# mrlooi/PoseCNN

Hardware: AMD Instinct MI355X
Metric: frames/sec 640x480x21-class Hough-vote+RoI+ADD-loss, 1/2/4/8 MI355X (higher is better)
Workload: dtype f32 (FC GEMMs: exact 3-way split-bf16 x6 MFMA, products within 2^-24, fp32 accumulate: fp32-faithful)

## Files before the change

include/posecnn_hip.h:

```cpp
#ifndef POSECNN_HIP_H
#define POSECNN_HIP_H

#include <stddef.h>
#include <stdint.h>

#ifdef __cplusplus
extern "C" {
#endif

#define PCNN_OK 0
#define PCNN_EINVAL 1
#define PCNN_EHIP 2
#define PCNN_ECAPACITY 3

#define PCNN_MAX_ROI 128

int pcnn_abi_version(void);
const char* pcnn_strerror(int code);

int pcnn_set_completion_event(void* event);
int pcnn_completion_event_pending(void);

size_t pcnn_hough_voting_workspace_size(int B, int H, int W, int C, int skip_pixels, float vote_thr);

// ... 36 lines not shown
                           float scale_b, int B, int C, const float* rois, int R_cap, int roi_stride,
                           int batch_base, const int32_t* num_rois_dev, int pooled_h, int pooled_w, float* top_sum,
                           int32_t* argmax_a, int32_t* argmax_b, void* stream);

int pcnn_roi_pool_fwd_pair_px(const float* data_a, int Ha, int Wa, float scale_a, const float* data_b, int Hb,
                              int Wb, float scale_b, int B, int C, const float* rois, int R_cap, int roi_stride,
                              int batch_base, const int32_t* num_rois_dev, int pooled_h, int pooled_w,
                              float* top_sum, uint16_t* argmax_a, uint16_t* argmax_b, void* stream);

size_t pcnn_roi_pool_bwd_workspace_size(int B, int R_cap);

int pcnn_roi_pool_bwd_form(int B, int H, int W, int C, int layout, int pool_channel, int pooled_h, int pooled_w,
                           int R_cap, int px);

int pcnn_roi_pool_bwd(const float* top_diff, const int32_t* argmax, int B, int H, int W, int C, int layout,
                      const float* rois, int R_cap, int roi_stride, int batch_base, const int32_t* num_rois_dev,
                      float spatial_scale, int pooled_h, int pooled_w, int pool_channel, float* bottom_diff,
                      void* workspace, size_t workspace_bytes, void* stream);

int pcnn_roi_pool_bwd_px(const float* top_diff, const uint16_t* argmax_px, int B, int H, int W, int C,
                         const float* rois, int R_cap, int roi_stride, int batch_base, const int32_t* num_rois_dev,
                         float spatial_scale, int pooled_h, int pooled_w, float* bottom_diff, void* workspace,
                         size_t workspace_bytes, void* stream);

size_t pcnn_add_loss_workspace_size(int R_cap, int C, int P);
size_t pcnn_add_loss_stats_offset(int R_cap, int C, int P);

int pcnn_add_loss_fwd(const float* pred, const float* target, const float* weight, const float* points,
                      const float* symmetry, int R_cap, const int32_t* num_rois_dev, int C, int P, float margin,
                      int loss_norm_rows, const int32_t* loss_norm_rows_dev, float* loss, float* bottom_diff,
                      void* workspace, size_t workspace_bytes, void* stream);

int pcnn_add_loss_prep(const float* weight, const float* symmetry, int R_cap, const int32_t* num_rois_dev, int C,
                       int P, void* workspace, size_t workspace_bytes, void* stream);
int pcnn_add_loss_fwd_prepared(const float* pred, const float* target, const float* weight, const float* points,
                               const float* symmetry, int R_cap, const int32_t* num_rois_dev, int C, int P,
                               float margin, int loss_norm_rows, const int32_t* loss_norm_rows_dev, float* loss,
                               float* bottom_diff, void* workspace, size_t workspace_bytes, void* stream);

int pcnn_add_loss_fwd_head_bwd(const float* pred, const float* target, const float* weight, const float* points,
                               const float* symmetry, int R_cap, const int32_t* num_rois_dev, int C, int P,
                               float margin, int loss_norm_rows, const int32_t* loss_norm_rows_dev,
                               float* bottom_diff, void* workspace, size_t workspace_bytes, const float* tanh_out,
                               const float* d_pred_scale, float* d_y8, void* stream);
int pcnn_add_loss_total(int R_cap, const int32_t* num_rois_dev, int C, int P, const void* workspace,
                        size_t workspace_bytes, float* loss, void* stream);
// ... 197 lines not shown
```

posecnn_amd/_lib.py:

```python
import ctypes
import os
import threading

import torch

_HERE = os.path.dirname(os.path.abspath(__file__))
LIB_PATH = os.environ.get("POSECNN_HIP_LIB") or os.path.join(_HERE, "libposecnn_hip.so")

_lib = None
_lock = threading.Lock()

c_int = ctypes.c_int
c_float = ctypes.c_float
c_size_t = ctypes.c_size_t
c_void_p = ctypes.c_void_p

_SIGS = {
    "pcnn_abi_version": (c_int, []),
    "pcnn_strerror": (ctypes.c_char_p, [c_int]),
    "pcnn_set_completion_event": (c_int, [c_void_p]),
    "pcnn_completion_event_pending": (c_int, []),
    "pcnn_hough_voting_workspace_size": (c_size_t, [c_int, c_int, c_int, c_int, c_int, c_float]),
    "pcnn_hough_voting": (c_int, [c_void_p, c_void_p, c_void_p, c_void_p, c_int, c_void_p, c_int, c_int, c_int,
                                  c_int, c_int, c_int, c_int, c_int, c_float, c_int, c_float, c_float, c_int,
# ... 5 lines not shown
                                       c_int, c_void_p, c_void_p, c_size_t, c_void_p]),
    "pcnn_hough_voting_compact": (c_int, [c_void_p, c_void_p, c_void_p, c_void_p, c_int, c_void_p, c_int, c_int,
                                          c_int, c_int, c_int, c_int, c_int, c_int, c_float, c_int, c_float, c_float,
                                          c_int, c_void_p, c_void_p, c_void_p, c_void_p, c_void_p, c_void_p, c_int,
                                          c_void_p, c_void_p, c_size_t, c_void_p]),
    "pcnn_hough_voting_grad": (c_int, [c_void_p, c_void_p, c_int, c_int, c_int, c_int, c_void_p]),
    "pcnn_hough_voting_diag": (c_int, [c_void_p, c_int, c_int, c_int, c_int, c_int, c_float, c_void_p, c_void_p]),
    "pcnn_roi_pool_fwd": (c_int, [c_void_p, c_int, c_int, c_int, c_int, c_int, c_void_p, c_int, c_int, c_int,
                                  c_void_p, c_float, c_int, c_int, c_int, c_void_p, c_void_p, c_void_p]),
    "pcnn_roi_pool_fwd_accumulate": (c_int, [c_void_p, c_int, c_int, c_int, c_int, c_int, c_void_p, c_int, c_int,
                                             c_int, c_void_p, c_float, c_int, c_int, c_int, c_void_p, c_void_p, c_void_p]),
    "pcnn_roi_pool_fwd_pair": (c_int, [c_void_p, c_int, c_int, c_float, c_void_p, c_int, c_int, c_float, c_int, c_int,
                                       c_void_p, c_int, c_int, c_int, c_void_p, c_int, c_int, c_void_p, c_void_p,
                                       c_void_p, c_void_p]),
    "pcnn_roi_pool_fwd_pair_px": (c_int, [c_void_p, c_int, c_int, c_float, c_void_p, c_int, c_int, c_float, c_int,
                                          c_int, c_void_p, c_int, c_int, c_int, c_void_p, c_int, c_int, c_void_p,
                                          c_void_p, c_void_p, c_void_p]),
    "pcnn_roi_pool_bwd_workspace_size": (c_size_t, [c_int, c_int]),
    "pcnn_roi_pool_bwd_form": (c_int, [c_int, c_int, c_int, c_int, c_int, c_int, c_int, c_int, c_int, c_int]),
    "pcnn_roi_pool_bwd_px": (c_int, [c_void_p, c_void_p, c_int, c_int, c_int, c_int, c_void_p, c_int, c_int, c_int,
                                     c_void_p, c_float, c_int, c_int, c_void_p, c_void_p, c_size_t, c_void_p]),
    "pcnn_roi_pool_bwd": (c_int, [c_void_p, c_void_p, c_int, c_int, c_int, c_int, c_int, c_void_p, c_int, c_int,
                                  c_int, c_void_p, c_float, c_int, c_int, c_int, c_void_p, c_void_p, c_size_t, c_void_p]),
    "pcnn_add_loss_workspace_size": (c_size_t, [c_int, c_int, c_int]),
    "pcnn_add_loss_stats_offset": (c_size_t, [c_int, c_int, c_int]),
    "pcnn_add_loss_fwd": (c_int, [c_void_p, c_void_p, c_void_p, c_void_p, c_void_p, c_int, c_void_p, c_int, c_int,
                                  c_float, c_int, c_void_p, c_void_p, c_void_p, c_void_p, c_size_t, c_void_p]),
    "pcnn_add_loss_fwd_prepared": (c_int, [c_void_p, c_void_p, c_void_p, c_void_p, c_void_p, c_int, c_void_p, c_int, c_int,
                                  c_float, c_int, c_void_p, c_void_p, c_void_p, c_void_p, c_size_t, c_void_p]),
    "pcnn_add_loss_prep": (c_int, [c_void_p, c_void_p, c_int, c_void_p, c_int, c_int, c_void_p, c_size_t, c_void_p]),
    "pcnn_add_loss_fwd_head_bwd": (c_int, [c_void_p, c_void_p, c_void_p, c_void_p, c_void_p, c_int, c_void_p, c_int,
                                           c_int, c_float, c_int, c_void_p, c_void_p, c_void_p, c_size_t, c_void_p,
                                           c_void_p, c_void_p, c_void_p]),
    "pcnn_add_loss_total": (c_int, [c_int, c_void_p, c_int, c_int, c_void_p, c_size_t, c_void_p, c_void_p]),
    "pcnn_add_loss_bwd": (c_int, [c_void_p, c_void_p, c_int, c_void_p, c_int, c_void_p, c_void_p]),
    "pcnn_div_rn_check": (c_int, [c_void_p, c_float, c_int, c_int, c_void_p, c_void_p]),
    "pcnn_backproject_fwd": (c_int, [c_void_p, c_void_p, c_void_p, c_void_p, c_int, c_void_p, c_int, c_int, c_int,
                                     c_int, c_int, c_int, c_int, c_float, c_void_p, c_void_p, c_void_p, c_void_p]),
    "pcnn_backproject_bwd": (c_int, [c_void_p, c_void_p, c_void_p, c_int, c_int, c_int, c_int, c_int, c_int,
                                     c_void_p, c_void_p]),
    "pcnn_gemm_workspace_size": (c_size_t, [c_int, c_int, c_int, c_int, c_int]),
    "pcnn_gemm": (c_int, [c_int, c_int, c_int, c_void_p, c_void_p, c_int, c_int, c_void_p, c_int, c_int, c_void_p,
                          c_int, c_void_p, c_int, c_void_p, c_int, c_void_p, c_void_p, c_int, c_void_p, c_size_t,
                          c_void_p]),
    "pcnn_gemm_drop": (c_int, [c_int, c_int, c_int, c_void_p, c_void_p, c_int, c_int, c_void_p, c_int, c_int,
                               c_void_p, c_int, c_void_p, c_int, c_void_p, c_int, c_void_p, c_int, c_float, c_void_p,
# ... 186 lines not shown
```

posecnn_amd/csrc/roi_plan.h:

```cpp
#pragma once

namespace pcnn_roi {

#ifndef PCNN_RBW_NARROW
#define PCNN_RBW_NARROW 8192
#endif
#ifndef PCNN_RBW_TH
#define PCNN_RBW_TH 2
#endif
static_assert(PCNN_RBW_TH == 1 || PCNN_RBW_TH == 2, "the entry-list forms are 1x4 and 2x4");

constexpr int kBWaves = 1;
constexpr int kBChunk = 128 * kBWaves;
constexpr int kBTileW = 4;
constexpr int kBGroup = 16;
constexpr int kBBins = 49;
constexpr int kBCap = kBGroup * kBBins;

enum BwdForm { kBwdRejected = -1, kBwdGeneric = 0, kBwdEnt1x4 = 1, kBwdEnt2x4 = 2 };

struct BwdPlan {
  int form;
  int tbh;
};
// ... 5 lines not shown
inline int bwd_tile_h(int B, int H, int W, int C) {
  const long nchunk = ((long)C + kBChunk - 1) / kBChunk;
  const long wg24 = (long)B * (((long)H + 1) / 2) * (((long)W + 3) / 4) * nchunk;
  return wg24 < PCNN_RBW_NARROW ? 1 : PCNN_RBW_TH;
}

inline BwdPlan bwd_plan(int B, int H, int W, int C, int layout, int pool_channel, int pooled_h, int pooled_w,
                        int R_cap, int px) {
  BwdPlan p = {kBwdRejected, 0};
  if (B <= 0 || H <= 0 || W <= 0 || C <= 0 || pooled_h <= 0 || pooled_w <= 0 || R_cap < 0 ||
      (layout != 0 && layout != 1) || !map_below(H, W, C, 1l << 31))
    return p;
  const int tbh = bwd_tile_h(B, H, W, C);
  const long bins = (long)pooled_h * pooled_w;
  const bool ent = layout == 0 && !pool_channel && C % 2 == 0 && (long)pooled_h * tbh <= 32 &&
                   (long)pooled_w * kBTileW <= 32 && kBGroup * bins <= kBCap && map_below(H, W, C, 1l << 30) &&
                   R_cap <= ((1l << 29) - 1) / (bins * C);
  if (px && !(ent && (long)H * W < 0xFFFF)) return p;
  p.form = !ent ? kBwdGeneric : tbh == 1 ? kBwdEnt1x4 : kBwdEnt2x4;
  p.tbh = ent ? tbh : 0;
  return p;
}

}
```

posecnn_amd/csrc/roi_pooling.hip:

```cpp
#include "pcnn_common.h"
#include "roi_plan.h"
#include <math.h>
#include <cfloat>

namespace {


struct RoiGeo {
  int b, cls, sw, sh, ew, eh;
  float bin_h, bin_w;
};

__device__ __forceinline__ RoiGeo roi_geo(const float* __restrict__ rois, int r, int stride, int batch_base,
                                          float scale, int PH, int PW) {
  const float* o = rois + (size_t)r * stride;
  RoiGeo g;
  g.b = (int)o[0] - batch_base;
  const int c0 = stride == 5 ? 1 : 2;
  g.cls = stride == 5 ? 0 : (int)o[1];
  g.sw = (int)roundf(o[c0 + 0] * scale);
  g.sh = (int)roundf(o[c0 + 1] * scale);
  g.ew = (int)roundf(o[c0 + 2] * scale);
  g.eh = (int)roundf(o[c0 + 3] * scale);
  const int roi_w = max(g.ew - g.sw + 1, 1);
// ... 365 lines not shown
        }
      };
      if (total > 0) {
        int2 myA, myB, avA[kBBatch], avB[kBBatch];
        float2 dvA[kBBatch], dvB[kBBatch];
        fetch(0, myA, avA, dvA);
        for (int e0 = 0; e0 < total; e0 += 2 * kBBatch) {
          if (e0 + kBBatch < total) fetch(e0 + kBBatch, myB, avB, dvB);
          accumulate(e0, myA, avA, dvA);
          if (e0 + 2 * kBBatch < total) fetch(e0 + 2 * kBBatch, myA, avA, dvA);
          if (e0 + kBBatch < total) accumulate(e0 + kBBatch, myB, avB, dvB);
        }
      }
      __syncthreads();
    }
  }
  if (cok) {
#pragma unroll
    for (int i = 0; i < kBTH; i++)
#pragma unroll
      for (int j = 0; j < kBTW; j++)
        if (i < th && j < tw) *(float2*)(bottom + (((size_t)b * H + h0 + i) * W + w0 + j) * C + c) = acc[i * kBTW + j];
  }
}

__global__ void k_roi_bwd_generic(const float* __restrict__ top_diff, const int32_t* __restrict__ argmax, int B,
                                  int H, int W, int C, int layout, const int32_t* __restrict__ geo, int PH, int PW,
                                  int pool_channel, const int32_t* __restrict__ lo, const int32_t* __restrict__ hi,
                                  float* __restrict__ bottom) {
  const long npix = (long)B * H * W;
  const int Co = pool_channel ? 1 : C;
  for (long pi = (long)blockIdx.x * blockDim.x + threadIdx.x; pi < npix; pi += (long)gridDim.x * blockDim.x) {
    const int w = (int)(pi % W), h = (int)((pi / W) % H), b = (int)(pi / ((long)W * H));
    const int r0 = lo[b], r1 = hi[b];
    for (int r = r0; r <= r1; r++) {
      const int32_t* gg = geo + (size_t)r * 8;
      RoiGeo g;
      g.b = gg[0]; g.cls = gg[1]; g.sw = gg[2]; g.sh = gg[3]; g.ew = gg[4]; g.eh = gg[5];
      g.bin_h = __int_as_float(gg[6]);
      g.bin_w = __int_as_float(gg[7]);
      if (g.b != b) continue;
      if (!(w >= g.sw && w <= g.ew && h >= g.sh && h <= g.eh)) continue;
      int phs, phe, pws, pwe;
      bins_of_pixel(g, h, w, PH, PW, phs, phe, pws, pwe);
      const int cb = pool_channel ? g.cls : 0, ce = pool_channel ? g.cls + 1 : C;
      if (cb < 0 || ce > C) continue;
// ... 162 lines not shown
    const int blocks = (int)((npix + 255) / 256 < 8192 ? (npix + 255) / 256 : 8192);
    hipLaunchKernelGGL(k_roi_bwd_generic, dim3(blocks), dim3(256), 0, st, top_diff, (const int32_t*)argmax, B, H, W,
                       C, layout, geo, pooled_h, pooled_w, pool_channel, lo, hi, bottom_diff);
  }
  PCNN_CHECK_LAUNCH();
  return PCNN_OK;
}

extern "C" int pcnn_roi_pool_bwd(const float* top_diff, const int32_t* argmax, int B, int H, int W, int C, int layout,
                                 const float* rois, int R_cap, int roi_stride, int batch_base,
                                 const int32_t* num_rois_dev, float spatial_scale, int pooled_h, int pooled_w,
                                 int pool_channel, float* bottom_diff, void* workspace, size_t workspace_bytes, void* stream) {
  return roi_pool_bwd(top_diff, argmax, false, B, H, W, C, layout, rois, R_cap, roi_stride, batch_base, num_rois_dev,
                      spatial_scale, pooled_h, pooled_w, pool_channel, bottom_diff, workspace, workspace_bytes, stream);
}

extern "C" int pcnn_roi_pool_bwd_px(const float* top_diff, const uint16_t* argmax_px, int B, int H, int W, int C,
                                    const float* rois, int R_cap, int roi_stride, int batch_base,
                                    const int32_t* num_rois_dev, float spatial_scale, int pooled_h, int pooled_w,
                                    float* bottom_diff, void* workspace, size_t workspace_bytes, void* stream) {
  return roi_pool_bwd(top_diff, argmax_px, true, B, H, W, C, 0, rois, R_cap, roi_stride, batch_base, num_rois_dev,
                      spatial_scale, pooled_h, pooled_w, 0, bottom_diff, workspace, workspace_bytes, stream);
}
```

posecnn_amd/pipeline.py:

```python
import contextlib

import torch

from . import _lib
from . import pose_head as ph
from .hough_voting_gpu_layer import hough_voting_gpu_op as hv
from .roi_pooling_layer import roi_pooling_op as rp
from .average_distance_loss import average_distance_loss_op as adl
from .exchange import GradShard, RoiExchange

CAP = hv.CAPACITY
_nullctx = contextlib.nullcontext


class PoseStep:
    def __init__(self, B, H, W, num_classes, device, conv4_hw=None, conv5_hw=None, channels=512, units=4096,
                 is_train=1, skip_pixels=10, vote_threshold=-1.0, vote_percentage=0.02, margin=0.01,
                 global_batch=None, batch_base=0, weights=None, dist=None, backward=True, precision=2,
                 overlap_weight_grads=True, pixel_argmax=True, keep_prob=None, drop_seed=0x5EED, side_prep=True,
                 drop_in_reduce=True, pipeline=False, prefetch_at="loss", fuse_loss_tail=True,
                 defer_side_join=False, signal_forks=True, pool_at_tail=False, fuse_fc8=True):
        self.B, self.H, self.W, self.C = B, H, W, num_classes
        self.dev = device
        self.is_train, self.skip, self.vthr, self.vper, self.margin = is_train, skip_pixels, vote_threshold, \
            vote_percentage, margin
        self.global_batch = global_batch or B
        self.batch_base = batch_base
        self.dist = dist
        self.backward = backward
        self.prec = precision
        self.h4, self.w4 = conv4_hw or (H // 8, W // 8)
        self.h5, self.w5 = conv5_hw or (H // 16, W // 16)
        self.Ch = channels
        D = 4 * num_classes
        self.D = D
        self.fuse_fc8 = bool(fuse_fc8) and dist is None and ph.fc8_fused_ok(units, D, precision) and D % 4 == 0
        self.weights = weights or ph.PoseHeadWeights(num_classes, device, in_dim=49 * channels, units=units)
        f32 = dict(dtype=torch.float32, device=device)
        i32 = dict(dtype=torch.int32, device=device)
        K6 = 49 * channels
        px = pixel_argmax and max(self.h4 * self.w4, self.h5 * self.w5) < 0xFFFF
        adt = dict(dtype=torch.int16 if px else torch.int32, device=device)

        def minibatch_set():
            return dict(hough=dict(box=torch.zeros((CAP, 7), **f32), pose=torch.zeros((CAP, 7), **f32),
                                   target=torch.zeros((CAP, D), **f32), weight=torch.zeros((CAP, D), **f32),
                                   domain=torch.zeros((CAP,), **i32), num_rois=torch.zeros((2,), **i32)),
                        pool=torch.zeros((CAP, 7, 7, channels), **f32),
                        arg5=torch.zeros((CAP, 7, 7, channels), **adt),
                        arg4=torch.zeros((CAP, 7, 7, channels), **adt),
                        add_ws=None, prepped=False)
        self.fuse_loss_tail = fuse_loss_tail
        self.pipeline = bool(pipeline)
        self._sets = [minibatch_set() for _ in range(2 if self.pipeline else 1)]
        self._cur = 0
        self._primed = None
        self.prefetch_at = prefetch_at
        if prefetch_at not in ("loss", "bwd", "start", "fwd", "tail"):
            raise ValueError("prefetch_at must be 'start', 'fwd', 'loss', 'bwd' or 'tail'")
        self._fork_ev = torch.cuda.Event() if self.pipeline else None
        self._fork_recorded = False
        self.pre_stream = torch.cuda.Stream(device=device) if self.pipeline else None
        self._next = None
        self.y6 = torch.zeros((CAP, units), **f32)
        self.y7 = torch.zeros((CAP, units), **f32)
        self.y8 = torch.zeros((CAP, D), **f32)
        self.t8 = torch.zeros((CAP, D), **f32)
        self.pred = torch.zeros((CAP, D), **f32)
        self.loss = torch.zeros((1,), **f32)
        self.diff = torch.zeros((CAP, D), **f32)
        self.one = torch.ones((1,), **f32)
        self.dy8 = torch.zeros((CAP, D), **f32)
        self.dy7 = torch.zeros((CAP, units), **f32)
        self.dy6 = torch.zeros((CAP, units), **f32)
        self.dx = torch.zeros((CAP, K6), **f32)
        self.gshard = None
        if dist is not None:
            per_max = 9 if is_train else 1
            slot = max(1, min(CAP, B * (hv.MAX_ROI // self.global_batch) * per_max))
            self.gshard = GradShard(dist, slot, [("w6", (K6, units)), ("w7", (units, units)), ("w8", (units, D))],
                                    device)
        self.grads = self.weights.grads_like()
        if self.gshard is not None:
            for k in ("w6", "w7", "w8"):
                self.grads[k] = self.grads[k][self.gshard.rows(k)].contiguous()
        self.keep = float(keep_prob if keep_prob is not None else (0.5 if is_train else 1.0))
# ... 105 lines not shown
        s = self._cur if s is None else s
        st = self._sets[s]
        if st["add_ws"] is None:
            st["add_ws"] = torch.empty(adl.workspace_bytes(CAP, self.C, points.shape[1]), dtype=torch.uint8,
                                       device=self.dev)
        h = st["hough"]
        side = None
        if stream is None:
            side = self.side_stream if self.timer is None and self.side_prep else None
            if side is not None:
                side.wait_stream(torch.cuda.current_stream())
        with torch.cuda.stream(stream or side or torch.cuda.current_stream()):
            adl.average_distance_loss_prep(h["weight"], symmetry, points.shape[1], st["add_ws"],
                                           num_rois=h["num_rois"][1:2])
        st["prepped"] = "side" if side is not None else "stream"

    def pool_fwd(self, conv4, conv5, s=None):
        s = self._cur if s is None else s
        st = self._sets[s]
        with self._t("roi_pool_fwd"):
            rp.roi_pool_pair(conv5, 1.0 / 16.0, conv4, 1.0 / 8.0, st["hough"]["box"], 7, 7,
                             num_rois=st["hough"]["num_rois"][1:2], out=(st["pool"], st["arg5"], st["arg4"]),
                             batch_base=self.batch_base)
        st["pooled"] = True

    def _front(self, inputs, s, stream=None):
        ctx = torch.cuda.stream(stream) if stream is not None else _nullctx()
        with ctx:
            self.vote(inputs["label"], inputs["vertex"], inputs["extents"], inputs["meta"], inputs["gt"], s=s)
            if stream is not None:
                self.add_prep(inputs["points"], inputs["symmetry"], s=s, stream=stream)
                if self.pool_at_tail and stream is self.pre_stream:
                    self._pool_pending = (inputs, s)
                else:
                    self.pool_fwd(inputs["conv4"], inputs["conv5"], s=s)

    def _issue_pending_pool(self):
        if self._pool_pending is None:
            return
        inputs, s = self._pool_pending
        self._pool_pending = None
        with torch.cuda.stream(self.pre_stream):
            self.pool_fwd(inputs["conv4"], inputs["conv5"], s=s)

    def _prefetch(self):
        if self._next is None:
# ... 185 lines not shown
        self._head_bwd_done = False
        if self.prefetch_at == "bwd":
            self._prefetch()
        with self._t("gemm_fc8_fc7_dw_bias"):
            weight_grads("w8", self.y7, self.dy8, CAP, w.units, self.D, fork=not fused_fork)
        dk = dict(keep_prob=self.keep) if self.keep < 1.0 else {}
        ev = self._arm_fork("fc8_dx") if side is not None else None
        with self._t("gemm_fc8_fc7_dx"):
            if self.fuse_fc8:
                self._timed_gemm("fc8_dx", lambda: ph.fc8_dx(self.dy8, w.w8, self.dy7, mask=self.y7, M_dev=nr,
                                                             precision=self.prec, **dk))
            else:
                self._g("fc8_dx", self.dy8, w.w8, self.dy7, b_trans=1, mask=self.y7, M_dev=nr, **dk)
        ev = self._fork_taken(ev)
        with self._t("gemm_fc8_fc7_dw_bias"):
            weight_grads("w7", self.y6, self.dy7, CAP, w.units, w.units, fork_ev=ev)
        defer = self.defer_side_join and side is not None
        self._side_wait("_side_done_ev")
        self._side_pending = False
        if defer:
            self._mid_covers_pre = (self._primed is not None and self._pool_pending is None and
                                    not torch.cuda.is_current_stream_capturing())
            if self._mid_covers_pre:
                side.wait_stream(self.pre_stream)
            if self._bump_drop_step and self._mid_covers_pre:
                with torch.cuda.stream(side):
                    self.drop_step.add_(1)
                self._bump_drop_step = False
            self._side_mid_ev.record(side)
        ev = self._arm_fork("fc7_dx") if side is not None else None
        with self._t("gemm_fc8_fc7_dx"):
            self._g("fc7_dx", self.dy7, w.w7, self.dy6, b_trans=1, mask=self.y6, M_dev=nr, **dk)
        ev = self._fork_taken(ev)
        with self._t("gemm_fc6_dw"):
            weight_grads("w6", x, self.dy6, CAP, K6, w.units, fork_ev=ev)
        with self._t("gemm_fc6_dx"):
            self._g("fc6_dx", self.dy6, w.w6, self.dx, b_trans=1, M_dev=nr)
        if self.prefetch_at == "tail":
            self._prefetch()
        self._issue_pending_pool()
        dxp = self.dx.view(CAP, 7, 7, self.Ch)
        with self._t("roi_pool_bwd"):
            rp.roi_pool_grad(conv5, h["box"], self.arg5, dxp, 7, 7, 1.0 / 16.0, 0, num_rois=nr, out=self.dconv5,
                             batch_base=self.batch_base)
            rp.roi_pool_grad(conv4, h["box"], self.arg4, dxp, 7, 7, 1.0 / 8.0, 0, num_rois=nr, out=self.dconv4,
                             batch_base=self.batch_base)
        if self._bump_drop_step:
            self.drop_step.add_(1)
            self._bump_drop_step = False
        if defer:
            self._side_done_ev.record(side)
            self._side_pending = True
        elif side is not None:
            main.wait_stream(side)

    def _g(self, name, A, B, C, **kw):
        self._timed_gemm(name, lambda: ph.gemm(A, B, C, precision=self.prec, **kw))
        return C

    def _timed_gemm(self, name, launch):
        if self.gemm_timer is None:
            return launch()
        e0, e1 = torch.cuda.Event(enable_timing=True), torch.cuda.Event(enable_timing=True)
        e0.record()
        out = launch()
        e1.record()
        self.gemm_timer.setdefault(name, []).append((e0, e1))
        return out

# ... 56 lines not shown
```

posecnn_amd/roi_pooling_layer/roi_pooling_op.py:

```python
import torch

from .. import _lib


def roi_pool(bottom_data, bottom_rois, pooled_height, pooled_width, spatial_scale, pool_channel=0, name=None,
             num_rois=None, layout=0, out=None, accumulate=False, batch_base=0):
    _lib.require_gpu(bottom_data, bottom_rois)
    if bottom_data.dim() != 4:
        raise ValueError("data must be 4-dimensional")
    if bottom_rois.dim() != 2:
        raise ValueError("rois must be 2-dimensional")
    data = bottom_data.contiguous().float()
    rois = bottom_rois.contiguous().float()
    if layout == 0:
        B, H, W, C = data.shape
    else:
        B, C, H, W = data.shape
    R, stride = rois.shape
    Co = 1 if pool_channel else C
    shape = (R, pooled_height, pooled_width, Co) if layout == 0 else (R, Co, pooled_height, pooled_width)
    if out is None:
        if accumulate:
            raise ValueError("accumulate=True needs out=(top, argmax)")
        top = torch.empty(shape, dtype=torch.float32, device=data.device)
# ... 53 lines not shown
    R, stride = rois.shape
    lib = _lib.load()
    ws = _lib.workspace(lib.pcnn_roi_pool_bwd_workspace_size(B, R), bottom_data.device, "roi_bwd")
    dd = out if out is not None else torch.empty(bottom_data.shape, dtype=torch.float32, device=bottom_data.device)
    px = argmax.dtype == torch.int16
    if R == 0:
        rois = argmax = grad = ws
    if px:
        if layout != 0 or pool_channel:
            raise ValueError("a pixel-index argmax needs NHWC data and pool_channel 0")
        rc = lib.pcnn_roi_pool_bwd_px(_lib.ptr(grad.contiguous()), _lib.ptr(argmax.contiguous()), B, H, W, C,
                                      _lib.ptr(rois), R, stride, int(batch_base), _lib.ptr(num_rois),
                                      float(spatial_scale), int(pooled_height), int(pooled_width), _lib.ptr(dd),
                                      _lib.ptr(ws), ws.numel(), _lib.stream_ptr())
    else:
        rc = lib.pcnn_roi_pool_bwd(_lib.ptr(grad.contiguous()), _lib.ptr(argmax.contiguous()), B, H, W, C, layout,
                                   _lib.ptr(rois), R, stride, int(batch_base), _lib.ptr(num_rois),
                                   float(spatial_scale), int(pooled_height), int(pooled_width), int(pool_channel),
                                   _lib.ptr(dd), _lib.ptr(ws), ws.numel(), _lib.stream_ptr())
    _lib.check(rc, "roi_pool_grad")
    return dd


class RoiPoolFunction(torch.autograd.Function):

    @staticmethod
    def forward(ctx, data, rois, pooled_height, pooled_width, spatial_scale, pool_channel=0, layout=0):
        top, arg = roi_pool(data, rois, pooled_height, pooled_width, spatial_scale, pool_channel, layout=layout)
        ctx.save_for_backward(data, rois, arg)
        ctx.params = (pooled_height, pooled_width, spatial_scale, pool_channel, layout)
        return top, arg

    @staticmethod
    def backward(ctx, grad, _garg):
        data, rois, arg = ctx.saved_tensors
        ph, pw, sc, pc, layout = ctx.params
        return roi_pool_grad(data, rois, arg, grad, ph, pw, sc, pc, layout=layout), None, None, None, None, None, None
```

Baseline: 4604.

## Precompute RoI-pool backward tile plan on prefetch stream and fuse conv4/conv5 backward

Adds a plan step that builds per-tile lists of intersecting RoIs with bin row and column bitmasks, using a count pass, a prefix scan and a fill pass. The step is issued after forward RoI pooling, on the prefetch stream when pipelining is on. The backward pass then walks only the precomputed records, skipping the per-tile RoI geometry scan, and runs conv4 and conv5 in a single paired launch with double-buffered loads. The cost is extra plan buffers, three small extra kernels per step and event synchronisation between streams; if the plan cannot be hidden on the side stream, it adds work to the step.

```diff
diff --git a/include/posecnn_hip.h b/include/posecnn_hip.h
--- a/include/posecnn_hip.h
+++ b/include/posecnn_hip.h
@@ -82,6 +82,20 @@
                          const float* rois, int R_cap, int roi_stride, int batch_base, const int32_t* num_rois_dev,
                          float spatial_scale, int pooled_h, int pooled_w, float* bottom_diff, void* workspace,
                          size_t workspace_bytes, void* stream);
+
+size_t pcnn_roi_pool_bwd_plan_bytes(int B, int H, int W, int C, int pooled_h, int pooled_w, int R_cap);
+int pcnn_roi_pool_bwd_plan(int B, int H, int W, int C, const float* rois, int R_cap, int roi_stride, int batch_base,
+                           const int32_t* num_rois_dev, float spatial_scale, int pooled_h, int pooled_w, void* plan,
+                           size_t plan_bytes, void* stream);
+
+int pcnn_roi_pool_bwd_planned(const float* top_diff, const void* argmax, int px, int B, int H, int W, int C,
+                              int R_cap, int pooled_h, int pooled_w, const void* plan, size_t plan_bytes,
+                              float* bottom_diff, void* stream);
+
+int pcnn_roi_pool_bwd_planned_pair(const float* top_diff, int px, int B, int C, int R_cap, int pooled_h, int pooled_w,
+                                   const void* argmax_a, int Ha, int Wa, const void* plan_a, size_t plan_a_bytes,
+                                   float* bottom_a, const void* argmax_b, int Hb, int Wb, const void* plan_b,
+                                   size_t plan_b_bytes, float* bottom_b, void* stream);
 
 size_t pcnn_add_loss_workspace_size(int R_cap, int C, int P);
 size_t pcnn_add_loss_stats_offset(int R_cap, int C, int P);
diff --git a/posecnn_amd/_lib.py b/posecnn_amd/_lib.py
--- a/posecnn_amd/_lib.py
+++ b/posecnn_amd/_lib.py
@@ -51,6 +51,14 @@
                                      c_void_p, c_float, c_int, c_int, c_void_p, c_void_p, c_size_t, c_void_p]),
     "pcnn_roi_pool_bwd": (c_int, [c_void_p, c_void_p, c_int, c_int, c_int, c_int, c_int, c_void_p, c_int, c_int,
                                   c_int, c_void_p, c_float, c_int, c_int, c_int, c_void_p, c_void_p, c_size_t, c_void_p]),
+    "pcnn_roi_pool_bwd_plan_bytes": (c_size_t, [c_int, c_int, c_int, c_int, c_int, c_int, c_int]),
+    "pcnn_roi_pool_bwd_plan": (c_int, [c_int, c_int, c_int, c_int, c_void_p, c_int, c_int, c_int, c_void_p, c_float,
+                                       c_int, c_int, c_void_p, c_size_t, c_void_p]),
+    "pcnn_roi_pool_bwd_planned": (c_int, [c_void_p, c_void_p, c_int, c_int, c_int, c_int, c_int, c_int, c_int, c_int,
+                                          c_void_p, c_size_t, c_void_p, c_void_p]),
+    "pcnn_roi_pool_bwd_planned_pair": (c_int, [c_void_p, c_int, c_int, c_int, c_int, c_int, c_int,
+                                               c_void_p, c_int, c_int, c_void_p, c_size_t, c_void_p,
+                                               c_void_p, c_int, c_int, c_void_p, c_size_t, c_void_p, c_void_p]),
     "pcnn_add_loss_workspace_size": (c_size_t, [c_int, c_int, c_int]),
     "pcnn_add_loss_stats_offset": (c_size_t, [c_int, c_int, c_int]),
     "pcnn_add_loss_fwd": (c_int, [c_void_p, c_void_p, c_void_p, c_void_p, c_void_p, c_int, c_void_p, c_int, c_int,
diff --git a/posecnn_amd/csrc/roi_plan.h b/posecnn_amd/csrc/roi_plan.h
--- a/posecnn_amd/csrc/roi_plan.h
+++ b/posecnn_amd/csrc/roi_plan.h
@@ -1,4 +1,7 @@
 #pragma once
+#include <math.h>
+#include <stddef.h>
+#include <stdint.h>
 
 namespace pcnn_roi {
 
@@ -51,4 +54,78 @@
   return p;
 }
 
+
+#if defined(__HIP__) || defined(__HIPCC__)
+#define PCNN_ROI_HD __host__ __device__
+#else
+#define PCNN_ROI_HD
+#endif
+
+PCNN_ROI_HD inline bool tile_hit(int sw, int sh, int ew, int eh, float bin_h, float bin_w, int h0, int w0, int th,
+                                 int tw, int tbh, int PH, int PW, uint32_t& rbits, uint32_t& cbits) {
+  rbits = 0;
+  cbits = 0;
+  if (!(sh <= h0 + th - 1 && eh >= h0 && sw <= w0 + tw - 1 && ew >= w0)) return false;
+  for (int i = 0; i < th; i++) {
+    const int h = h0 + i;
+    if (h < sh || h > eh) continue;
+    int s0 = (int)floorf((float)(h - sh) / bin_h), e0 = (int)ceilf((float)(h - sh + 1) / bin_h);
+    s0 = s0 < 0 ? 0 : (s0 > PH ? PH : s0);
+    e0 = e0 < 0 ? 0 : (e0 > PH ? PH : e0);
+    for (int ph = s0; ph < e0; ph++) rbits |= 1u << (ph * tbh + i);
+  }
+  for (int j = 0; j < tw; j++) {
+    const int w = w0 + j;
+    if (w < sw || w > ew) continue;
+    int s0 = (int)floorf((float)(w - sw) / bin_w), e0 = (int)ceilf((float)(w - sw + 1) / bin_w);
+    s0 = s0 < 0 ? 0 : (s0 > PW ? PW : s0);
+    e0 = e0 < 0 ? 0 : (e0 > PW ? PW : e0);
+    for (int pw = s0; pw < e0; pw++) cbits |= 1u << (pw * kBTileW + j);
+  }
+  return rbits != 0 && cbits != 0;
 }
+
+constexpr int kPlanRowBits = 20;
+PCNN_ROI_HD inline uint64_t plan_pack(uint32_t r, uint32_t rbits, uint32_t cbits, int rb, int cb) {
+  return (uint64_t)cbits | ((uint64_t)rbits << cb) | ((uint64_t)r << (cb + rb));
+}
+PCNN_ROI_HD inline void plan_unpack(uint64_t rec, int rb, int cb, uint32_t& r, uint32_t& rbits, uint32_t& cbits) {
+  cbits = (uint32_t)(rec & ((1ull << cb) - 1));
+  rbits = (uint32_t)((rec >> cb) & ((1ull << rb) - 1));
+  r = (uint32_t)(rec >> (cb + rb));
+}
+
+constexpr int kPlanMagic = 0x524f4950;
+constexpr int kPlanHdr = 8;
+
+struct PlanLayout {
+  int ok, tbh;
+  long tpi, tiles, cap;
+  size_t hdr, lo, hi, geo, off, rec, bytes;
+};
+
+inline size_t plan_align(size_t x) { return (x + 255) / 256 * 256; }
+
+inline PlanLayout plan_layout(int B, int H, int W, int C, int pooled_h, int pooled_w, int R_cap) {
+  PlanLayout L = {};
+  const BwdPlan p = bwd_plan(B, H, W, C, 0, 0, pooled_h, pooled_w, R_cap, 0);
+  if (p.form != kBwdEnt1x4 && p.form != kBwdEnt2x4) return L;
+  if (R_cap >= (1 << kPlanRowBits) || pooled_h * p.tbh + pooled_w * kBTileW + kPlanRowBits > 64) return L;
+  L.tbh = p.tbh;
+  L.tpi = (((long)H + p.tbh - 1) / p.tbh) * (((long)W + kBTileW - 1) / kBTileW);
+  L.tiles = (long)B * L.tpi;
+  L.cap = (long)R_cap * L.tpi;
+  if (L.cap >= (1l << 31) || L.tiles >= (1l << 31) - 1) return L;
+  size_t o = 0;
+  L.hdr = o; o = plan_align(o + kPlanHdr * 4);
+  L.lo = o;  o = plan_align(o + (size_t)B * 4);
+  L.hi = o;  o = plan_align(o + (size_t)B * 4);
+  L.geo = o; o = plan_align(o + (size_t)(R_cap > 0 ? R_cap : 1) * 32);
+  L.off = o; o = plan_align(o + (size_t)(L.tiles + 1) * 4);
+  L.rec = o; o = plan_align(o + (size_t)(L.cap > 0 ? L.cap : 1) * 8);
+  L.bytes = o;
+  L.ok = 1;
+  return L;
+}
+
+}
diff --git a/posecnn_amd/csrc/roi_pooling.hip b/posecnn_amd/csrc/roi_pooling.hip
--- a/posecnn_amd/csrc/roi_pooling.hip
+++ b/posecnn_amd/csrc/roi_pooling.hip
@@ -411,6 +411,232 @@
       for (int j = 0; j < kBTW; j++)
         if (i < th && j < tw) *(float2*)(bottom + (((size_t)b * H + h0 + i) * W + w0 + j) * C + c) = acc[i * kBTW + j];
   }
+}
+
+
+template <bool FILL>
+__global__ void __launch_bounds__(256) k_roi_plan_tiles(const int32_t* __restrict__ geo,
+                                                         const int32_t* __restrict__ lo,
+                                                         const int32_t* __restrict__ hi, int H, int W, int tbh,
+                                                         int PH, int PW, int tpi, int tiles,
+                                                         int32_t* __restrict__ off, uint64_t* __restrict__ recs) {
+  const int tile = (int)blockIdx.x * 4 + (int)(threadIdx.x >> 6);
+  if (tile >= tiles) return;
+  const int lane = pcnn::lane_id();
+  const int tiles_w = (W + pcnn_roi::kBTileW - 1) / pcnn_roi::kBTileW;
+  const int b = tile / tpi, t = tile % tpi;
+  const int h0 = (t / tiles_w) * tbh, w0 = (t % tiles_w) * pcnn_roi::kBTileW;
+  const int th = min(tbh, H - h0), tw = min(pcnn_roi::kBTileW, W - w0);
+  const int r0 = lo[b], r1 = hi[b];
+  const int base = FILL ? off[tile] : 0;
+  int n = 0;
+  for (int rb = r0; rb <= r1; rb += 64) {
+    const int r = rb + lane;
+    uint32_t rbits = 0, cbits = 0;
+    bool hit = false;
+    if (r <= r1) {
+      const int32_t* gg = geo + (size_t)r * 8;
+      if (gg[0] == b)
+        hit = pcnn_roi::tile_hit(gg[2], gg[3], gg[4], gg[5], __int_as_float(gg[6]), __int_as_float(gg[7]), h0, w0, th,
+                                 tw, tbh, PH, PW, rbits, cbits);
+    }
+    const uint64_t hits = __ballot(hit);
+    if (FILL && hit)
+      recs[(size_t)base + n + __popcll(hits & pcnn::lanemask_lt())] =
+          pcnn_roi::plan_pack((uint32_t)r, rbits, cbits, PH * tbh, PW * pcnn_roi::kBTileW);
+    n += __popcll(hits);
+  }
+  if (!FILL && lane == 0) off[tile] = n;
+}
+
+__global__ void __launch_bounds__(1024) k_roi_plan_scan(int32_t* __restrict__ off, int tiles, int32_t* __restrict__ hdr,
+                                                         int B, int H, int W, int tbh, int PH, int PW, int R_cap) {
+  __shared__ int wsum[16];
+  const int lane = pcnn::lane_id(), wave = threadIdx.x >> 6;
+  int carry = 0;
+  for (int t0 = 0; t0 < tiles; t0 += 1024) {
+    const int i = t0 + (int)threadIdx.x;
+    const int v = i < tiles ? off[i] : 0;
+    int s = v;
+#pragma unroll
+    for (int d = 1; d < 64; d <<= 1) {
+      const int u = __shfl_up(s, d, 64);
+      if (lane >= d) s += u;
+    }
+    if (lane == 63) wsum[wave] = s;
+    __syncthreads();
+    int before = 0, total = 0;
+#pragma unroll
+    for (int k = 0; k < 16; k++) {
+      const int ws = wsum[k];
+      before += k < wave ? ws : 0;
+      total += ws;
+    }
+    if (i < tiles) off[i] = carry + before + s - v;
+    carry += total;
+    __syncthreads();
+  }
+  if (threadIdx.x == 0) {
+    off[tiles] = carry;
+    hdr[0] = pcnn_roi::kPlanMagic; hdr[1] = B; hdr[2] = H; hdr[3] = W;
+    hdr[4] = tbh; hdr[5] = PH; hdr[6] = PW; hdr[7] = R_cap;
+  }
+}
+
+struct PlanMap {
+  const void* argmax;
+  const int32_t* hdr;
+  const int32_t* off;
+  const uint64_t* recs;
+  float* bottom;
+  int H, W;
+  int items;
+  int ipx;
+};
+
+template <int kBTH, bool PX>
+__device__ __forceinline__ void roi_bwd_planned_tile(const float* __restrict__ top_diff, int B, int C, int PH, int PW,
+                                                     int R_cap, const PlanMap& pm, int bid) {
+  constexpr int kBTW = pcnn_roi::kBTileW, kBPix = kBTH * kBTW;
+  const int H = pm.H, W = pm.W;
+  const int tiles_w = (W + kBTW - 1) / kBTW, tiles_h = (H + kBTH - 1) / kBTH;
+  const int tpi = tiles_w * tiles_h;
+  const int nchunk = (C + kBChunk - 1) / kBChunk;
+  int id = (bid % 8) * pm.ipx + bid / 8;
+  if (id >= pm.items) return;
+  const int chunk = id % nchunk;
+  const int tile = id / nchunk;
+  const int t = tile % tpi, b = tile / tpi;
+  const int h0 = (t / tiles_w) * kBTH, w0 = (t % tiles_w) * kBTW;
+  const int th = min(kBTH, H - h0), tw = min(kBTW, W - w0);
+  const int lane = pcnn::lane_id();
+  const int c = chunk * kBChunk + 2 * lane;
+  const bool cok = c < C;
+  float2 acc[kBPix];
+  int expv[kBPix];
+#pragma unroll
+  for (int p = 0; p < kBPix; p++) {
+    acc[p] = make_float2(0.f, 0.f);
+    const int pix = (h0 + p / kBTW) * W + w0 + p % kBTW;
+    expv[p] = PX ? pix : pix * C + c;
+  }
+  constexpr int kNext = PX ? 0 : 1;
+  const int4 hd0 = *(const int4*)pm.hdr, hd1 = *(const int4*)(pm.hdr + 4);
+  const bool built = ((hd0.x ^ pcnn_roi::kPlanMagic) | (hd0.y ^ B) | (hd0.z ^ H) | (hd0.w ^ W) | (hd1.x ^ kBTH) |
+                      (hd1.y ^ PH) | (hd1.z ^ PW) | (hd1.w ^ R_cap)) == 0;
+  const int e_lo = pm.off[tile], e_hi = pm.off[tile + 1];
+  const long cap = (long)R_cap * tpi;
+  const int n = built && e_lo >= 0 && e_hi >= e_lo && (long)e_hi <= cap ? e_hi - e_lo : 0;
+  const uint64_t* recs = pm.recs + e_lo;
+  const int bins = PH * PW, rb = PH * kBTH, cb = PW * kBTW;
+  const bool lane_bin = lane < bins;
+  const int rsh = lane_bin ? (lane / PW) * kBTH : 0, csh = lane_bin ? (lane % PW) * kBTW : 0;
+  const __amdgpu_buffer_rsrc_t rs_t = __builtin_amdgcn_make_buffer_rsrc((void*)top_diff, (short)0, 0x7fffffff, 0x00020000);
+  const __amdgpu_buffer_rsrc_t rs_a = __builtin_amdgcn_make_buffer_rsrc((void*)pm.argmax, (short)0, 0x7fffffff, 0x00020000);
+  const unsigned voff = cok ? (unsigned)c * 4u : 0x80000000u;
+  const unsigned voff_a = cok ? (unsigned)c * (PX ? 2u : 4u) : 0x80000000u;
+  int i = 0;
+  uint64_t valid = 0;
+  int mvec = 0;
+  int ebase = 0;
+  uint64_t myrec = 0;
+  auto list = [&](int2& my) -> int {
+    int k = 0;
+    while (k < kBBatch) {
+      if (valid == 0) {
+        if (i >= n) break;
+        if ((i & 63) == 0) myrec = i + lane < n ? recs[i + lane] : 0;
+        const uint32_t w0r = (uint32_t)__builtin_amdgcn_readlane((int)(uint32_t)myrec, i & 63);
+        const uint32_t w1r = (uint32_t)__builtin_amdgcn_readlane((int)(uint32_t)(myrec >> 32), i & 63);
+        i++;
+        uint32_t r, rbits, cbits;
+        pcnn_roi::plan_unpack((uint64_t)w0r | ((uint64_t)w1r << 32), rb, cb, r, rbits, cbits);
+        const uint32_t rm = (rbits >> rsh) & ((1u << kBTH) - 1), cm = (cbits >> csh) & ((1u << kBTW) - 1);
+        uint32_t m = 0;
+#pragma unroll
+        for (int q = 0; q < kBTH; q++)
+          if ((rm >> q) & 1) m |= cm << (q * kBTW);
+        mvec = lane_bin ? (int)m : 0;
+        valid = (int)r < R_cap ? __ballot(mvec != 0) : 0;
+        ebase = (int)r * bins * C;
+        continue;
+      }
+      const int l = __builtin_ctzll(valid);
+      valid &= valid - 1;
+      const int em = __builtin_amdgcn_readlane(mvec, l);
+      if (lane == k) my = make_int2(ebase + l * C, em);
+      k++;
+    }
+    return k;
+  };
+  auto fetch = [&](const int2& my, int2 (&av)[kBBatch], float2 (&dv)[kBBatch]) {
+#pragma unroll
+    for (int k = 0; k < kBBatch; k++) {
+      const int so = __builtin_amdgcn_readlane(my.x, k) * 4;
+      if (PX)
+        av[k].x = (int)__builtin_amdgcn_raw_buffer_load_b32(rs_a, voff_a, so >> 1, 0);
+      else
+        av[k] = __builtin_bit_cast(int2, __builtin_amdgcn_raw_buffer_load_b64(rs_a, voff_a, so, 0));
+      dv[k] = __builtin_bit_cast(float2, __builtin_amdgcn_raw_buffer_load_b64(rs_t, voff, so, 0));
+    }
+  };
+  auto accumulate = [&](int cnt, const int2& my, const int2 (&av)[kBBatch], const float2 (&dv)[kBBatch]) {
+#pragma unroll
+    for (int k = 0; k < kBBatch; k++) {
+      if (k >= cnt) break;
+      const uint32_t m = (uint32_t)__builtin_amdgcn_readlane(my.y, k);
+      const int ax = PX ? (int)((unsigned)av[k].x & 0xFFFFu) : av[k].x;
+      const int ay = PX ? (int)((unsigned)av[k].x >> 16) : av[k].y;
+#pragma unroll
+      for (int q = 0; q < kBPix; q++) {
+        if (!((m >> q) & 1)) continue;
+        asm volatile("");
+        acc[q].x += ax == expv[q] ? dv[k].x : 0.f;
+        acc[q].y += ay == expv[q] + kNext ? dv[k].y : 0.f;
+      }
+    }
+  };
+  int2 myA = make_int2(0, 0), myB = make_int2(0, 0);
+  int2 avA[kBBatch], avB[kBBatch];
+  float2 dvA[kBBatch], dvB[kBBatch];
+  int cntA = list(myA);
+  if (cntA > 0) {
+    fetch(myA, avA, dvA);
+    for (;;) {
+      const int cntB = list(myB);
+      if (cntB == 0) {
+        accumulate(cntA, myA, avA, dvA);
+        break;
+      }
+      fetch(myB, avB, dvB);
+      accumulate(cntA, myA, avA, dvA);
+      cntA = list(myA);
+      if (cntA == 0) {
+        accumulate(cntB, myB, avB, dvB);
+        break;
+      }
+      fetch(myA, avA, dvA);
+      accumulate(cntB, myB, avB, dvB);
+    }
+  }
+  if (cok) {
+#pragma unroll
+    for (int i2 = 0; i2 < kBTH; i2++)
+#pragma unroll
+      for (int j = 0; j < kBTW; j++)
+        if (i2 < th && j < tw)
+          *(float2*)(pm.bottom + (((size_t)b * H + h0 + i2) * W + w0 + j) * C + c) = acc[i2 * kBTW + j];
+  }
+}
+
+template <int kTHA, int kTHB, bool PX>
+__global__ void __launch_bounds__(64) k_roi_bwd_planned(const float* __restrict__ top_diff, int B, int C, int PH,
+                                                        int PW, int R_cap, PlanMap ma, PlanMap mb, int na) {
+  const int bid = (int)blockIdx.x;
+  if (bid < na)
+    roi_bwd_planned_tile<kTHA, PX>(top_diff, B, C, PH, PW, R_cap, ma, bid);
+  else
+    roi_bwd_planned_tile<kTHB, PX>(top_diff, B, C, PH, PW, R_cap, mb, bid - na);
 }
 
 __global__ void k_roi_bwd_generic(const float* __restrict__ top_diff, const int32_t* __restrict__ argmax, int B,
@@ -619,3 +845,104 @@
   return roi_pool_bwd(top_diff, argmax_px, true, B, H, W, C, 0, rois, R_cap, roi_stride, batch_base, num_rois_dev,
                       spatial_scale, pooled_h, pooled_w, 0, bottom_diff, workspace, workspace_bytes, stream);
 }
+
+
+extern "C" size_t pcnn_roi_pool_bwd_plan_bytes(int B, int H, int W, int C, int pooled_h, int pooled_w, int R_cap) {
+  return pcnn_roi::plan_layout(B, H, W, C, pooled_h, pooled_w, R_cap).bytes;
+}
+
+extern "C" int pcnn_roi_pool_bwd_plan(int B, int H, int W, int C, const float* rois, int R_cap, int roi_stride,
+                                      int batch_base, const int32_t* num_rois_dev, float spatial_scale, int pooled_h,
+                                      int pooled_w, void* plan, size_t plan_bytes, void* stream) {
+  const pcnn_roi::PlanLayout L = pcnn_roi::plan_layout(B, H, W, C, pooled_h, pooled_w, R_cap);
+  PCNN_REQUIRE(L.ok && rois && plan && roi_stride >= 5 && ((uintptr_t)plan & 7) == 0);
+  if (plan_bytes < L.bytes) return PCNN_ECAPACITY;
+  hipStream_t st = (hipStream_t)stream;
+  char* p = (char*)plan;
+  int32_t* hdr = (int32_t*)(p + L.hdr);
+  int32_t* lo = (int32_t*)(p + L.lo);
+  int32_t* hi = (int32_t*)(p + L.hi);
+  int32_t* geo = (int32_t*)(p + L.geo);
+  int32_t* off = (int32_t*)(p + L.off);
+  uint64_t* recs = (uint64_t*)(p + L.rec);
+  const int tiles = (int)L.tiles, tpi = (int)L.tpi;
+  const unsigned nwg = (unsigned)((tiles + 3) / 4);
+  hipLaunchKernelGGL(k_roi_prep, dim3(1), dim3(1024), 0, st, rois, R_cap, roi_stride, batch_base, num_rois_dev, B,
+                     spatial_scale, pooled_h, pooled_w, geo, lo, hi);
+  hipLaunchKernelGGL(k_roi_plan_tiles<false>, dim3(nwg), dim3(256), 0, st, geo, lo, hi, H, W, L.tbh, pooled_h,
+                     pooled_w, tpi, tiles, off, recs);
+  hipLaunchKernelGGL(k_roi_plan_scan, dim3(1), dim3(1024), 0, st, off, tiles, hdr, B, H, W, L.tbh, pooled_h, pooled_w,
+                     R_cap);
+  pcnn::launch_last(k_roi_plan_tiles<true>, dim3(nwg), dim3(256), 0, st, geo, lo, hi, H, W, L.tbh, pooled_h, pooled_w,
+                    tpi, tiles, off, recs);
+  PCNN_CHECK_LAUNCH();
+  return PCNN_OK;
+}
+
+static int plan_map(const void* argmax, int px, int B, int H, int W, int C, int R_cap, int pooled_h, int pooled_w,
+                    const void* plan, size_t plan_bytes, float* bottom, PlanMap* pm, int* tbh) {
+  const pcnn_roi::PlanLayout L = pcnn_roi::plan_layout(B, H, W, C, pooled_h, pooled_w, R_cap);
+  PCNN_REQUIRE(L.ok && argmax && plan && bottom && (!px || (long)H * W < 0xFFFF));
+  PCNN_REQUIRE(((uintptr_t)bottom & 7) == 0 && ((uintptr_t)argmax & (px ? 3 : 7)) == 0 && ((uintptr_t)plan & 7) == 0);
+  if (plan_bytes < L.bytes) return PCNN_ECAPACITY;
+  const long items = L.tiles * (((long)C + kBChunk - 1) / kBChunk);
+  PCNN_REQUIRE(items < (1l << 30));
+  const char* p = (const char*)plan;
+  pm->argmax = argmax;
+  pm->hdr = (const int32_t*)(p + L.hdr);
+  pm->off = (const int32_t*)(p + L.off);
+  pm->recs = (const uint64_t*)(p + L.rec);
+  pm->bottom = bottom;
+  pm->H = H;
+  pm->W = W;
+  pm->items = (int)items;
+  pm->ipx = (int)((items + 7) / 8);
+  *tbh = L.tbh;
+  return PCNN_OK;
+}
+
+static int roi_pool_bwd_planned(const float* top_diff, int px, int B, int C, int R_cap, int pooled_h, int pooled_w,
+                                const PlanMap& ma, int tha, const PlanMap* mb, int thb, void* stream) {
+  PCNN_REQUIRE(top_diff && ((uintptr_t)top_diff & 7) == 0);
+  const int na = ma.ipx * 8, nb = mb ? mb->ipx * 8 : 0;
+  const PlanMap b = mb ? *mb : ma;
+  hipStream_t st = (hipStream_t)stream;
+#define PCNN_RBP(TA, TB, PXV)                                                                                     \
+  pcnn::launch_last(k_roi_bwd_planned<TA, TB, PXV>, dim3((unsigned)(na + nb)), dim3(64), 0, st, top_diff, B, C, \
+                    pooled_h, pooled_w, R_cap, ma, b, na)
+#define PCNN_RBP_PX(TA, TB) \
+  do { if (px) PCNN_RBP(TA, TB, true); else PCNN_RBP(TA, TB, false); } while (0)
+  if (tha == 2 && thb == 2) PCNN_RBP_PX(2, 2);
+  else if (tha == 2) PCNN_RBP_PX(2, 1);
+  else if (thb == 2) PCNN_RBP_PX(1, 2);
+  else PCNN_RBP_PX(1, 1);
+#undef PCNN_RBP_PX
+#undef PCNN_RBP
+  PCNN_CHECK_LAUNCH();
+  return PCNN_OK;
+}
+
+extern "C" int pcnn_roi_pool_bwd_planned(const float* top_diff, const void* argmax, int px, int B, int H, int W, int C,
+                                         int R_cap, int pooled_h, int pooled_w, const void* plan, size_t plan_bytes,
+                                         float* bottom_diff, void* stream) {
+  PlanMap ma;
+  int tha;
+  const int rc = plan_map(argmax, px, B, H, W, C, R_cap, pooled_h, pooled_w, plan, plan_bytes, bottom_diff, &ma, &tha);
+  if (rc != PCNN_OK) return rc;
+  return roi_pool_bwd_planned(top_diff, px, B, C, R_cap, pooled_h, pooled_w, ma, tha, nullptr, tha, stream);
+}
+
+extern "C" int pcnn_roi_pool_bwd_planned_pair(const float* top_diff, int px, int B, int C, int R_cap, int pooled_h,
+                                              int pooled_w, const void* argmax_a, int Ha, int Wa, const void* plan_a,
+                                              size_t plan_a_bytes, float* bottom_a, const void* argmax_b, int Hb,
+                                              int Wb, const void* plan_b, size_t plan_b_bytes, float* bottom_b,
+                                              void* stream) {
+  PlanMap ma, mb;
+  int tha, thb;
+  int rc = plan_map(argmax_a, px, B, Ha, Wa, C, R_cap, pooled_h, pooled_w, plan_a, plan_a_bytes, bottom_a, &ma, &tha);
+  if (rc != PCNN_OK) return rc;
+  rc = plan_map(argmax_b, px, B, Hb, Wb, C, R_cap, pooled_h, pooled_w, plan_b, plan_b_bytes, bottom_b, &mb, &thb);
+  if (rc != PCNN_OK) return rc;
+  PCNN_REQUIRE((long)ma.ipx * 8 + (long)mb.ipx * 8 < (1l << 31));
+  return roi_pool_bwd_planned(top_diff, px, B, C, R_cap, pooled_h, pooled_w, ma, tha, &mb, thb, stream);
+}
diff --git a/posecnn_amd/pipeline.py b/posecnn_amd/pipeline.py
--- a/posecnn_amd/pipeline.py
+++ b/posecnn_amd/pipeline.py
@@ -41,6 +41,13 @@
         K6 = 49 * channels
         px = pixel_argmax and max(self.h4 * self.w4, self.h5 * self.w5) < 0xFFFF
         adt = dict(dtype=torch.int16 if px else torch.int32, device=device)
+        u8 = dict(dtype=torch.uint8, device=device)
+
+        def plan_bytes(h, w):
+            n = rp.roi_pool_plan_bytes((B, h, w, channels), 7, 7, CAP)
+            if n == 0:
+                raise ValueError(f"PoseStep: the planned RoI-pool backward does not take a {h}x{w}x{channels} map")
+            return n
 
         def minibatch_set():
             return dict(hough=dict(box=torch.zeros((CAP, 7), **f32), pose=torch.zeros((CAP, 7), **f32),
@@ -49,6 +56,8 @@
                         pool=torch.zeros((CAP, 7, 7, channels), **f32),
                         arg5=torch.zeros((CAP, 7, 7, channels), **adt),
                         arg4=torch.zeros((CAP, 7, 7, channels), **adt),
+                        plan5=torch.zeros(plan_bytes(self.h5, self.w5), **u8) if backward else None,
+                        plan4=torch.zeros(plan_bytes(self.h4, self.w4), **u8) if backward else None,
                         add_ws=None, prepped=False)
         self.fuse_loss_tail = fuse_loss_tail
         self.pipeline = bool(pipeline)
@@ -62,6 +71,9 @@
         self._fork_recorded = False
         self.pre_stream = torch.cuda.Stream(device=device) if self.pipeline else None
         self._next = None
+        self._pre_front_ev = torch.cuda.Event() if self.pipeline else None
+        self._pre_front_recorded = False
+        self._plan_evs = [torch.cuda.Event() for _ in self._sets]
         self.y6 = torch.zeros((CAP, units), **f32)
         self.y7 = torch.zeros((CAP, units), **f32)
         self.y8 = torch.zeros((CAP, D), **f32)
@@ -213,6 +225,21 @@
             rp.roi_pool_pair(conv5, 1.0 / 16.0, conv4, 1.0 / 8.0, st["hough"]["box"], 7, 7,
                              num_rois=st["hough"]["num_rois"][1:2], out=(st["pool"], st["arg5"], st["arg4"]),
                              batch_base=self.batch_base)
+        st["plan_ev"] = None
+        if st["plan5"] is not None:
+            ahead = (self.pre_stream is not None and self.timer is None and
+                     torch.cuda.current_stream() == self.pre_stream and
+                     not torch.cuda.is_current_stream_capturing())
+            if ahead:
+                self._pre_front_ev.record(self.pre_stream)
+            self._pre_front_recorded = ahead
+            with self._t("roi_pool_bwd_plan"):
+                for key, hw, scale in (("plan4", (self.h4, self.w4), 1.0 / 8.0), ("plan5", (self.h5, self.w5), 1.0 / 16.0)):
+                    rp.roi_pool_plan((self.B,) + hw + (self.Ch,), st["hough"]["box"], 7, 7, scale,
+                                     num_rois=st["hough"]["num_rois"][1:2], batch_base=self.batch_base, out=st[key])
+            if ahead:
+                st["plan_ev"] = self._plan_evs[s]
+                st["plan_ev"].record(self.pre_stream)
         st["pooled"] = True
 
     def _front(self, inputs, s, stream=None):
@@ -444,7 +471,10 @@
             self._mid_covers_pre = (self._primed is not None and self._pool_pending is None and
                                     not torch.cuda.is_current_stream_capturing())
             if self._mid_covers_pre:
-                side.wait_stream(self.pre_stream)
+                if self._pre_front_recorded:
+                    side.wait_event(self._pre_front_ev)
+                else:
+                    side.wait_stream(self.pre_stream)
             if self._bump_drop_step and self._mid_covers_pre:
                 with torch.cuda.stream(side):
                     self.drop_step.add_(1)
@@ -462,11 +492,18 @@
             self._prefetch()
         self._issue_pending_pool()
         dxp = self.dx.view(CAP, 7, 7, self.Ch)
+        st = self._sets[self._cur]
         with self._t("roi_pool_bwd"):
-            rp.roi_pool_grad(conv5, h["box"], self.arg5, dxp, 7, 7, 1.0 / 16.0, 0, num_rois=nr, out=self.dconv5,
-                             batch_base=self.batch_base)
-            rp.roi_pool_grad(conv4, h["box"], self.arg4, dxp, 7, 7, 1.0 / 8.0, 0, num_rois=nr, out=self.dconv4,
-                             batch_base=self.batch_base)
+            if st["plan5"] is not None:
+                if st.get("plan_ev") is not None and not torch.cuda.is_current_stream_capturing():
+                    main.wait_event(st["plan_ev"])
+                rp.roi_pool_grad_planned_pair(CAP, dxp, 7, 7, self.arg4, st["plan4"], self.dconv4,
+                                              self.arg5, st["plan5"], self.dconv5)
+            else:
+                rp.roi_pool_grad(conv5, h["box"], self.arg5, dxp, 7, 7, 1.0 / 16.0, 0, num_rois=nr, out=self.dconv5,
+                                 batch_base=self.batch_base)
+                rp.roi_pool_grad(conv4, h["box"], self.arg4, dxp, 7, 7, 1.0 / 8.0, 0, num_rois=nr, out=self.dconv4,
+                                 batch_base=self.batch_base)
         if self._bump_drop_step:
             self.drop_step.add_(1)
             self._bump_drop_step = False
diff --git a/posecnn_amd/roi_pooling_layer/roi_pooling_op.py b/posecnn_amd/roi_pooling_layer/roi_pooling_op.py
--- a/posecnn_amd/roi_pooling_layer/roi_pooling_op.py
+++ b/posecnn_amd/roi_pooling_layer/roi_pooling_op.py
@@ -99,6 +99,62 @@
     return dd
 
 
+def roi_pool_plan_bytes(data_shape, pooled_height, pooled_width, rows):
+    B, H, W, C = data_shape
+    return int(_lib.load().pcnn_roi_pool_bwd_plan_bytes(B, H, W, C, int(pooled_height), int(pooled_width), int(rows)))
+
+
+def roi_pool_plan(data_shape, bottom_rois, pooled_height, pooled_width, spatial_scale, num_rois=None, batch_base=0,
+                  out=None):
+    _lib.require_gpu(bottom_rois)
+    B, H, W, C = data_shape
+    rois = bottom_rois.contiguous().float()
+    R, stride = rois.shape
+    nbytes = roi_pool_plan_bytes(data_shape, pooled_height, pooled_width, R)
+    if nbytes == 0:
+        raise ValueError("roi_pool_plan: the planned backward does not take this shape")
+    plan = out if out is not None else torch.empty(nbytes, dtype=torch.uint8, device=rois.device)
+    if R == 0:
+        rois = plan
+    rc = _lib.load().pcnn_roi_pool_bwd_plan(B, H, W, C, _lib.ptr(rois), R, stride, int(batch_base), _lib.ptr(num_rois),
+                                            float(spatial_scale), int(pooled_height), int(pooled_width),
+                                            _lib.ptr(plan), plan.numel(), _lib.stream_ptr())
+    _lib.check(rc, "roi_pool_plan")
+    return plan
+
+
+def roi_pool_grad_planned(data_shape, rows, argmax, grad, pooled_height, pooled_width, plan, out=None):
+    _lib.require_gpu(argmax, grad, plan)
+    B, H, W, C = data_shape
+    dd = out if out is not None else torch.empty(tuple(data_shape), dtype=torch.float32, device=plan.device)
+    px = argmax.dtype == torch.int16
+    if rows == 0:
+        argmax = grad = plan
+    rc = _lib.load().pcnn_roi_pool_bwd_planned(_lib.ptr(grad.contiguous()), _lib.ptr(argmax.contiguous()), int(px), B,
+                                               H, W, C, int(rows), int(pooled_height), int(pooled_width),
+                                               _lib.ptr(plan), plan.numel(), _lib.ptr(dd), _lib.stream_ptr())
+    _lib.check(rc, "roi_pool_grad_planned")
+    return dd
+
+
+def roi_pool_grad_planned_pair(rows, grad, pooled_height, pooled_width, argmax_a, plan_a, out_a, argmax_b, plan_b,
+                               out_b):
+    _lib.require_gpu(grad, argmax_a, plan_a, out_a, argmax_b, plan_b, out_b)
+    B, Ha, Wa, C = out_a.shape
+    Bb, Hb, Wb, Cb = out_b.shape
+    if (Bb, Cb) != (B, C) or argmax_a.dtype != argmax_b.dtype:
+        raise ValueError("both maps need the same batch, channel count and argmax form")
+    px = argmax_a.dtype == torch.int16
+    if rows == 0:
+        argmax_a = argmax_b = grad = plan_a
+    rc = _lib.load().pcnn_roi_pool_bwd_planned_pair(
+        _lib.ptr(grad.contiguous()), int(px), B, C, int(rows), int(pooled_height), int(pooled_width),
+        _lib.ptr(argmax_a.contiguous()), Ha, Wa, _lib.ptr(plan_a), plan_a.numel(), _lib.ptr(out_a),
+        _lib.ptr(argmax_b.contiguous()), Hb, Wb, _lib.ptr(plan_b), plan_b.numel(), _lib.ptr(out_b), _lib.stream_ptr())
+    _lib.check(rc, "roi_pool_grad_planned_pair")
+    return out_a, out_b
+
+
 class RoiPoolFunction(torch.autograd.Function):
 
     @staticmethod
```

Result: no change. 4581 (-0.5%).
